# ERGO-Code/ipx

Hardware: AMD Instinct MI355X
Metric: kkt_solves_per_sec (higher is better)
Workload: dtype f64; 1 GPU; C3 synthetic LP m=1000000 n=2000000 8 nnz/col (nnz=16000000), KKTSolverDiag::Solve = diag-precond CR to tol=0.3*sqrt(mu), scaling spread s=1; rows of AI partitioned over 1 GPU(s); errflag=0

## Files before the change

include/ipx_kkt_hip.h:

```cpp
#ifndef IPX_KKT_HIP_H_
#define IPX_KKT_HIP_H_

#include <stdint.h>

#ifdef __cplusplus
extern "C" {
#endif

typedef int64_t ipxint;
typedef struct ipxk_context ipxk_context;

#define IPXK_OK 0
#define IPXK_E_HIP (-1)
#define IPXK_E_ALLOC (-2)
#define IPXK_E_ARGUMENT (-3)
#define IPXK_E_UNSUPPORTED (-4)

#define IPXK_POINTER_HOST 0
#define IPXK_POINTER_DEVICE 1

#define IPXK_NONBASIC_FIXED (-2)
#define IPXK_NONBASIC (-1)
#define IPXK_BASIC 0
#define IPXK_BASIC_FREE 1
// ... 50 lines not shown
int ipxk_get_reorder_info(const ipxk_context* ctx, ipxk_reorder_info* info);
int ipxk_get_reordering(ipxk_context* ctx, ipxint* rowperm, ipxint* colperm);
int ipxk_get_rowwise(const ipxk_context* ctx, ipxint* ATp, ipxint* ATi,
                     double* ATx);

int ipxk_normal_prepare(ipxk_context* ctx, const double* W);
int ipxk_normal_apply(ipxk_context* ctx, const double* rhs, double* lhs,
                      double* rhs_dot_lhs);

int ipxk_diag_factorize(ipxk_context* ctx, const double* W,
                        int precond_dense_cols, ipxint* errflag);
int ipxk_diag_apply(ipxk_context* ctx, const double* rhs, double* lhs,
                    double* rhs_dot_lhs);
int ipxk_diag_get(const ipxk_context* ctx, double* diagonal, double* chol);

typedef ipxint (*ipxk_interrupt_fn)(void* user);
int ipxk_pcr_solve(ipxk_context* ctx, const double* rhs, double tol,
                   const double* resscale, ipxint maxiter, double* lhs,
                   ipxint* iter, ipxint* errflag, ipxk_interrupt_fn interrupt,
                   void* interrupt_user, double* resnorm_hist, ipxint hist_cap,
                   ipxk_times* times);

int ipxk_cr_diagnostics(ipxk_context* ctx, ipxk_cr_diag* out);

int ipxk_kkt_diag_factorize(ipxk_context* ctx, const double* xl,
                            const double* xu, const double* zl,
                            const double* zu, double mu,
                            int precond_dense_cols, ipxint* errflag);
int ipxk_kkt_diag_solve(ipxk_context* ctx, const double* a, const double* b,
                        double tol, ipxint maxiter, double* x, double* y,
                        ipxint* iter, ipxint* errflag,
                        ipxk_interrupt_fn interrupt, void* interrupt_user,
                        ipxk_times* times);
int ipxk_kkt_diag_get(const ipxk_context* ctx, double* W, double* resscale);

int ipxk_split_prepare(ipxk_context* ctx, const ipxint* Lp, const ipxint* Li,
                       const double* Lx, const ipxint* Up, const ipxint* Ui,
                       const double* Ux, const ipxint* rowperm,
                       const ipxint* colperm, const ipxint* basis,
                       const ipxint* status, const double* colscale);
int ipxk_split_rescale(ipxk_context* ctx, const ipxint* status,
                       const double* colscale);
typedef struct {
  ipxint lnz, unz;
  ipxint num_dependent;
  ipxint col_singletons, row_singletons, bump, rounds;
// ... 262 lines not shown
```

ipx_amd/csrc/api.hip:

```cpp

#include <algorithm>
#include <map>
#include <thread>

#include "context.hpp"

namespace ipxk {

static thread_local std::string g_last_error;
void set_last_error(const std::string& msg) { g_last_error = msg; }

Context::~Context() {
    if (split) destroy_split(split);
    if (split_spare) destroy_split(split_spare);
    if (prepare_host) destroy_prepare_host(prepare_host);
    if (lu) destroy_lu(lu);
    if (maxvol) destroy_maxvol(maxvol);
    if (nmat) destroy_nmatrix(nmat);
    comm_destroy(this);
    if (h_state) (void)hipHostFree(h_state);
    if (h_cycle_done) (void)hipHostFree(h_cycle_done);
    if (ev_a) (void)hipEventDestroy(ev_a);
    if (ev_b) (void)hipEventDestroy(ev_b);
    for (hipEvent_t e : ev_window) (void)hipEventDestroy(e);
// ... 1008 lines not shown
        IPXK_REQUIRE(!comm_active(c), kDeviceLuRefusal);
        bind_device(c);
        maxvolume_dev(c, status, colscale, params, basis_out, status_out, info, exchange_log, log_cap);
    });
}

int ipxk_maxvolume_sequential(ipxk_context* c, const ipxint* status, const double* colscale, double volume_tol, ipxint maxpasses,
                              ipxint max_etas, ipxint* basis_out, ipxint* status_out, ipxk_maxvolume_info* info,
                              ipxint* exchange_log, ipxint log_cap) {
    return guarded([&] {
        IPXK_REQUIRE(c && status && colscale, "NULL argument");
        IPXK_REQUIRE(log_cap >= 0 && (exchange_log || log_cap == 0), "bad log arguments");
        IPXK_REQUIRE(!comm_active(c), kDeviceLuRefusal);
        bind_device(c);
        maxvolume_sequential_dev(c, status, colscale, volume_tol, maxpasses, max_etas, basis_out, status_out, info, exchange_log, log_cap);
    });
}

int ipxk_cr_diagnostics(ipxk_context* c, ipxk_cr_diag* out) {
    return guarded([&] {
        IPXK_REQUIRE(c && out, "NULL argument");
        bind_device(c);
        cr_diagnostics_dev(c, out);
    });
}

int ipxk_split_rescale(ipxk_context* c, const ipxint* status, const double* colscale) {
    return guarded([&] {
        IPXK_REQUIRE(c && status && colscale, "NULL argument");
        IPXK_REQUIRE(c->split != nullptr, "SplittedNormalMatrix not prepared");
        bind_device(c);
        split_rescale_host(c, status, colscale);
    });
}

int ipxk_split_apply(ipxk_context* c, const double* rhs, double* lhs, double* rhs_dot_lhs) {
    return guarded([&] {
        IPXK_REQUIRE(c && rhs && lhs, "NULL argument");
        IPXK_REQUIRE(c->split != nullptr, "SplittedNormalMatrix not prepared");
        split_check_partition(c);
        bind_device(c);
        if (c->partials.size() == 0) c->partials.resize((size_t)kNumPartialSlots * kPartialStride);
        const size_t m = (size_t)c->m;
        const double* drhs = stage_in(c, rhs, m, c->v_rhs);
        double* dlhs = stage_out(c, lhs, m, c->v_lhs);
        const int np = split_apply_dev(c, drhs, dlhs, nullptr);
// ... 264 lines not shown
```

ipx_amd/csrc/context.hpp:

```cpp
#pragma once

#include "internal.hpp"
#include "device_utils.hpp"

struct ncclComm;

namespace ipxk {

constexpr int kPartialStride = kMaxPartials + 8;

enum PartialSlot {
    kPartRes0 = 0,
    kPartRes1,
    kPartPdot,
    kPartCdot,
    kPartRsdot,
    kPartScratch,
    kNumPartialSlots
};

struct Reordered {
    bool active = false;
    int levels = 0;
    int components = 0;
// ... 49 lines not shown

    DevBuf<double> diagonal;
    bool diag_factorized = false;
    int64_t kdense = 0;
    GatherMatrix AdCols;
    GatherMatrix AdRows;
    DevBuf<double> chol, chol_inv, smw_work, smw_u, Wnodense;
    DevBuf<double> schur_panel, schur_part;
    DevBuf<int> schur_colptr;
    DevBuf<int> chol_info;
    DevBuf<unsigned char> dense_mask;
    std::vector<int> dense_rank_k;
    DevBuf<double> dense_W, dense_Wsend, dense_Wrecv;
    DevBuf<int> dense_Widx;

    DevBuf<double> v_rhs, v_lhs, v_residual, v_sresidual, v_step, v_Cstep, v_Cres, v_pCstep;
    DevBuf<double> v_resscale_in;
    DevBuf<double> partials;
    DevBuf<CrState> state;
    CrState* h_state = nullptr;
    DevBuf<double> hist;
    hipEvent_t ev_a = nullptr, ev_b = nullptr;
    std::vector<hipEvent_t> ev_window;

    DevBuf<double> resscale;
    DevBuf<double> k_a, k_b, k_x, k_y;
    DevBuf<double> k_tmp;
    bool kkt_diag_factorized = false;

    DevBuf<double> nw_rhs1, nw_rhs2;
    DevBuf<double> nw_in[10], nw_out[6];
    DevBuf<unsigned char> nw_state;

    DevBuf<double> it_x, it_xl, it_xu, it_y, it_zl, it_zu, it_partials;
    DevBuf<double> it_row, it_bnd, it_table;
    DevBuf<unsigned char> it_state;
    bool it_set = false;
    DevBuf<double> ipm[12];
    bool postprocessed = false;
    double crossover_start = 0.0;
    DevBuf<double> colmax;
    bool have_colmax = false;

    struct { long inverse_probes = 0, inverse_rejected = 0, inverse_refined = 0; double worst_probe = 0.0; } split_stats;
    SplitOperator* split = nullptr;
    SplitOperator* split_spare = nullptr;
// ... 57 lines not shown
void reorder_permute_rows(Context* c, const double* in_old, double* out_new);
void reorder_unpermute_rows(Context* c, const double* in_new, double* out_old);
void reorder_permute_weights(Context* c, const double* W_old, double* W_new);

void dense_lu_inverse(Context* c, int kb, const double* D, const double* invL, const double* invU, double* X, double* Xt, int refine = 0);

enum TimeKind { kTimeOp = 0, kTimePrecond = 1, kTimeB = 2, kTimeBt = 3, kNumTimeKinds = 4 };
void time_mark(Context* c, int kind, bool begin);
void time_start(Context* c, ipxk_times* times);
void time_collect(Context* c, ipxk_times* times);

const double* stage_in(Context* c, const double* p, size_t len, DevBuf<double>& buf);
double* stage_out(Context* c, double* p, size_t len, DevBuf<double>& buf);
void finish_out(Context* c, double* user, const double* dev, size_t len);

void normal_apply_dev(Context* c, const double* W, const double* rhs, double* lhs, int* ndot,
                      const int* done);
float time_normal_pair(Context* c, GatherMatrix& Ac, GatherMatrix& Ar);
void debug_single_pass(Context* c, int which, const double* x, double* out);

void prepare_dense_columns(Context* c);
void reset_dense_columns(Context* c);
void diag_factorize_dev(Context* c, const double* W, bool precond_dense_cols, ipxint* errflag);
int diag_apply_dev(Context* c, const double* rhs, double* lhs, int slot, const int* done);

struct CrResult { ipxint iter; ipxint errflag; };
CrResult pcr_solve_dev(Context* c, const double* rhs, double tol, const double* resscale,
                       ipxint maxiter, double* lhs, bool lhs_is_zero, ipxk_interrupt_fn interrupt,
                       void* user, double* hist_host, ipxint hist_cap, ipxk_times* times);
CrResult cr_solve_dev(Context* c, const double* rhs, double tol, const double* resscale,
                      ipxint maxiter, double* lhs, bool lhs_is_zero, ipxk_interrupt_fn interrupt,
                      void* user, double* hist_host, ipxint hist_cap, ipxk_times* times);
double reduce_partials_host(Context* c, int slot, int count, bool is_max);
void cr_diagnostics_dev(Context* c, ipxk_cr_diag* out);
struct PartRef publish_scalar(Context* c, int slot, int count, int op);
struct PartRef allreduce_scalar(Context* c, int slot, int count, int op);

CrResult newton_solve_dev(Context* c, bool use_basis, const double* rb, const double* rc, const double* rl,
                          const double* ru, const double* sl, const double* su, const double* xl, const double* xu,
                          const double* zl, const double* zu, const unsigned char* state, double tol,
                          ipxint maxiter, double* dx, double* dxl, double* dxu, double* dy, double* dzl,
                          double* dzu, ipxk_interrupt_fn interrupt, void* user, ipxk_times* times);

void iterate_update_dev(Context* c, double sp, const double* dx, const double* dxl, const double* dxu, double sd,
                        const double* dy, const double* dzl, const double* dzu);
void iterate_residuals_dev(Context* c, const double* b, const double* cc, const double* lb, const double* ub,
                           double* rb, double* rc, double* rl, double* ru, double* presidual, double* dresidual);
void iterate_complementarity_dev(Context* c, double out4[4], double* num_terms = nullptr);
enum IterWhat : unsigned { kIterResiduals = 1, kIterComplementarity = 2, kIterObjectives = 4 };
struct IterScalars {
    double presidual = 0, dresidual = 0;
    double comp[4] = {0, 0, 0, 0};
    double num_terms = 0;
    double obj[3] = {0, 0, 0};
};
void iterate_scalars_dev(Context* c, unsigned what, const double* b, const double* cc, const double* lb, const double* ub,
                         double* rb, double* rc, double* rl, double* ru, IterScalars* out);
// ... 155 lines not shown
```

ipx_amd/csrc/cr.hip:

```cpp
#include <cmath>

#include "context.hpp"
#include "spmv_kernels.hpp"

namespace ipxk {

constexpr int kWindow = 2;

enum CrMode { kModePcrDiag = 0, kModePcrSmw = 1, kModePlain = 2 };

constexpr int kCrUnroll = 4;

struct CrVecs {
    int m;
    double* lhs;
    double* residual;
    double* sresidual;
    double* step;
    double* Cstep;
    double* Cres;
    double* pCstep;
    const double* resscale;
    const double* diag;
};

__global__ __launch_bounds__(kBlock) void residual_init_kernel(int m, const double* __restrict__ rhs,
                                                               const double* __restrict__ sub,
                                                               const double* __restrict__ resscale,
                                                               double* __restrict__ out,
                                                               double* partial) {
// ... 160 lines not shown
    }

    double mx = 0.0;
    long long i0 = first;
    if (EARLY) {
        ctl_update<MODE>(v, lazy, alpha, i0, stride, last, g0, mx);
        i0 += kCrUnroll * stride;
    }
    for (; i0 < v.m; i0 += kCrUnroll * stride) {
        CtlGroup g{};
        ctl_load<MODE>(v, lazy, i0, stride, last, g);
        ctl_update<MODE>(v, lazy, alpha, i0, stride, last, g, mx);
    }
    mx = block_reduce<MaxOp>(mx, red);
    if (threadIdx.x == 0) ((k & 1) ? res_next0 : res_next1)[blockIdx.x] = mx;
    if (writer) {
        st->k_started = k + 1;
        st->resnorm = resnorm;
        if (lazy) { st->alpha_pending = alpha; st->k_pending = k; }
    }
}

struct DirGroup {
    double p[kCrUnroll], q[kCrUnroll], s[kCrUnroll], cs[kCrUnroll], d[kCrUnroll], l[kCrUnroll];
};
template <int MODE, bool INIT>
__device__ __forceinline__ void dir_load(const CrVecs& v, const double* src, bool with_lhs, long long i0, long long stride,
                                         long long last, DirGroup& g) {
#pragma unroll
    for (int u = 0; u < kCrUnroll; u++) {
        const long long i = min(i0 + u * stride, last);
        g.p[u] = src[i];
        g.q[u] = v.Cres[i];
        if (!INIT) { g.s[u] = v.step[i]; g.cs[u] = v.Cstep[i]; }
        if (MODE == kModePcrDiag) g.d[u] = v.diag[i];
        if (!INIT && with_lhs) g.l[u] = v.lhs[i];
    }
}
template <int MODE, bool INIT>
__device__ __forceinline__ void dir_update(const CrVecs& v, bool owed, double alpha, double beta, long long i0, long long stride,
                                           long long last, DirGroup& g, double& acc) {
#pragma unroll
    for (int u = 0; u < kCrUnroll; u++) {
        const long long i = i0 + u * stride;
        if (i > last) break;
        if (!INIT) {
            if (owed) v.lhs[i] = g.l[u] + alpha * g.s[u];
            g.p[u] = g.p[u] + beta * g.s[u];
            g.q[u] = g.q[u] + beta * g.cs[u];
        }
        v.step[i] = g.p[u];
        v.Cstep[i] = g.q[u];
        if (MODE == kModePcrDiag) acc += (g.q[u] / g.d[u]) * g.q[u];
        if (MODE == kModePlain) acc += g.q[u] * g.q[u];
    }
}

template <int MODE, bool INIT, bool EARLY>
__global__ __launch_bounds__(kBlock) void cr_direction_kernel(CrState* st, CrVecs v, PartRef cdot_ref,
                                                              double* pdot_partial) {
    __shared__ double red[kBlock / 64 + 1];
    const double* src = MODE == kModePlain ? v.residual : v.sresidual;
    const long long stride = (long long)gridDim.x * kBlock, last = v.m - 1;
    const long long first = blockIdx.x * kBlock + threadIdx.x;
    long long k;
    double cdotnew, beta, alpha;
    bool owed;
    DirGroup g0{};
    if (EARLY) {
        const int done = st->done;
        const long long k_started = st->k_started, k_pending = st->k_pending;
        const double cdot0 = st->cdot[0], cdot1 = st->cdot[1];
        alpha = st->alpha_pending;
        double pc[kPartialsPerThread];
        load_partials(cdot_ref, pc);
        dir_load<MODE, INIT>(v, src, true, first, stride, last, g0);
        cdotnew = block_reduce<SumOp>(fold_partials<SumOp>(cdot_ref, pc), red);
        if (done) return;
        k = INIT ? -1 : k_started - 1;
        beta = INIT ? 0.0 : cdotnew / ((k & 1) ? cdot1 : cdot0);
        owed = !INIT && k_pending == k;
    } else {
        if (st->done) return;
        k = INIT ? -1 : st->k_started - 1;
        cdotnew = reduce_partials<SumOp>(cdot_ref, red);
        beta = INIT ? 0.0 : cdotnew / st->cdot[k & 1];
        owed = !INIT && st->k_pending == k;
        alpha = st->alpha_pending;
    }
    double acc = 0.0;
    long long i0 = first;
    if (EARLY) {
        dir_update<MODE, INIT>(v, owed, alpha, beta, i0, stride, last, g0, acc);
        i0 += kCrUnroll * stride;
    }
    for (; i0 < v.m; i0 += kCrUnroll * stride) {
        DirGroup g{};
        dir_load<MODE, INIT>(v, src, owed, i0, stride, last, g);
        dir_update<MODE, INIT>(v, owed, alpha, beta, i0, stride, last, g, acc);
    }
    if (MODE != kModePcrSmw) {
        acc = block_reduce<SumOp>(acc, red);
        if (threadIdx.x == 0) pdot_partial[blockIdx.x] = acc;
    }
    if (blockIdx.x == 0 && threadIdx.x == 0) {
        st->cdot[(k + 1) & 1] = cdotnew;
        st->k_finished = k + 1;
    }
}

__global__ __launch_bounds__(kBlock) void cr_flush_update_kernel(const CrState* st, CrVecs v) {
    if (st->k_pending < 0 || st->k_pending != st->k_finished) return;
    const double alpha = st->alpha_pending;
    for (int i = blockIdx.x * kBlock + threadIdx.x; i < v.m; i += gridDim.x * kBlock) v.lhs[i] += alpha * v.step[i];
}

__global__ __launch_bounds__(kBlock) void finalize_scalar_kernel(PartRef ref, int op, double* out) {
    __shared__ double red[kBlock / 64 + 1];
    const double v = op == 1 ? reduce_partials<MaxOp>(ref, red)
                   : op == 2 ? reduce_partials<MinOp>(ref, red) : reduce_partials<SumOp>(ref, red);
    if (threadIdx.x == 0) *out = v;
}

__global__ void snapshot_done_kernel(const CrState* st, int* host_slot) {
    __hip_atomic_store(host_slot, st->done, __ATOMIC_RELAXED, __HIP_MEMORY_SCOPE_SYSTEM);
}
__global__ void cycle_flags_kernel(const CrState* st, double interrupt_flag, double* flags) {
    flags[0] = (double)st->done;
    flags[1] = interrupt_flag;
}
__global__ void snapshot_flags_kernel(const double* flags, int* host_done, int* host_interrupt) {
    __hip_atomic_store(host_interrupt, (int)flags[1], __ATOMIC_RELAXED, __HIP_MEMORY_SCOPE_SYSTEM);
    __hip_atomic_store(host_done, (int)flags[0], __ATOMIC_RELAXED, __HIP_MEMORY_SCOPE_SYSTEM);
}

constexpr int kDoneRing = kWindow + 2;
constexpr int kDoneNow = 2 * kDoneRing;

static bool cr_lazy() {
    static const bool setting = [] { const char* e = getenv("IPXK_CR_LAZY"); return !e || atoi(e) != 0; }();
    return setting;
}

static bool cr_early() {
    static const bool setting = [] { const char* e = getenv("IPXK_CR_EARLY"); return !e || atoi(e) != 0; }();
    return setting;
}

static int cr_grid_cap() {
    static const int setting = [] { const char* e = getenv("IPXK_CR_GRID"); return e ? atoi(e) : 0; }();
    return setting;
}

static void ensure_comm_buffers(Context* c) {
    if (c->comm_scalars.size() < 64) c->comm_scalars.resize(64);
    if (c->comm_send.size() < (size_t)kNumPartialSlots) {
        c->comm_send.resize(kNumPartialSlots);
        IPXK_HIP(hipMemsetAsync(c->comm_send.get(), 0, sizeof(double) * kNumPartialSlots, c->stream));
    }
    const size_t need = (size_t)c->nranks * kNumPartialSlots;
// ... 66 lines not shown
        IPXK_HIP(hipHostGetDevicePointer(reinterpret_cast<void**>(&c->d_cycle_done), c->h_cycle_done, 0));
    }
    while ((int)c->ev_window.size() < kWindow + 1) {
        hipEvent_t e;
        IPXK_HIP(hipEventCreateWithFlags(&e, hipEventDisableTiming));
        c->ev_window.push_back(e);
    }
}

struct CrOps {
    int mode;
    int (*applyC)(Context*, const double* rhs, double* lhs, const int* done);
};

static int applyC_normal(Context* c, const double* rhs, double* lhs, const int* done) {
    int np = 0;
    time_mark(c, kTimeOp, true);
    normal_apply_dev(c, c->W, rhs, lhs, &np, done);
    time_mark(c, kTimeOp, false);
    return np;
}
static int applyC_split(Context* c, const double* rhs, double* lhs, const int* done) {
    return split_apply_dev(c, rhs, lhs, done);
}

template <int MODE>
static CrResult run_cr(Context* c, const CrOps& ops, const double* rhs, double tol,
                       const double* resscale, ipxint maxiter, double* lhs, bool lhs_is_zero,
                       ipxk_interrupt_fn interrupt, void* user, double* hist_host, ipxint hist_cap,
                       ipxk_times* times) {
    ensure_workspaces(c);
    time_start(c, times);
    hipStream_t s = c->stream;
    const int m = (int)c->m;
    if (maxiter < 0) maxiter = (comm_active(c) ? c->m_global : c->m) + 100;
    if (hist_cap < 0) hist_cap = 0;
    if (!hist_host) hist_cap = 0;
    if (c->hist.size() < (size_t)hist_cap + 1) c->hist.resize((size_t)hist_cap + 1);
    CrState* st = c->state.get();
    int* done = &st->done;
    const int g = cr_grid_cap() > 0 ? std::min(vec_grid(m), cr_grid_cap()) : vec_grid(m);
    const Pub pub(c);
    for (int i = 0; i <= kDoneNow; i++) c->h_cycle_done[i] = 0;
    const bool multi = comm_active(c);
    const int lazy = cr_lazy() ? 1 : 0;
    const bool early = cr_early() && m > 0;
    const auto control = early ? cr_control_update_kernel<MODE, true> : cr_control_update_kernel<MODE, false>;
    const auto direction0 = early ? cr_direction_kernel<MODE, true, true> : cr_direction_kernel<MODE, true, false>;
    const auto direction = early ? cr_direction_kernel<MODE, false, true> : cr_direction_kernel<MODE, false, false>;
    int* done_now = multi ? nullptr : c->d_cycle_done + kDoneNow;
    if (multi) ensure_comm_buffers(c);

    CrVecs v;
    v.m = m; v.lhs = lhs; v.residual = c->v_residual.get(); v.sresidual = c->v_sresidual.get();
    v.step = c->v_step.get(); v.Cstep = c->v_Cstep.get(); v.Cres = c->v_Cres.get();
    v.pCstep = c->v_pCstep.get(); v.resscale = resscale; v.diag = c->reord.in_use ? c->reord.diagonal.get() : c->diagonal.get();

    IPXK_HIP(hipEventRecord(c->ev_a, s));

    if (lhs_is_zero) {
        hipLaunchKernelGGL(residual_init_kernel, dim3(g), dim3(kBlock), 0, s, m, rhs,
                           (const double*)nullptr, resscale, v.residual, c->part(kPartRes0));
    } else {
        ops.applyC(c, lhs, v.Cres, nullptr);
        hipLaunchKernelGGL(residual_init_kernel, dim3(g), dim3(kBlock), 0, s, m, rhs,
                           (const double*)v.Cres, resscale, v.residual, c->part(kPartRes0));
    }
    int nrsdot = 0;
    if (MODE != kModePlain) nrsdot = diag_apply_dev(c, v.residual, v.sresidual, kPartRsdot, nullptr);
    if (MODE != kModePlain) pub.publish(kPartRes0, g, 1, kPartRsdot, nrsdot, 0);
    else pub.publish(kPartRes0, g, 1);
    const PartRef res0 = pub.ref(kPartRes0, g), res1 = pub.ref(kPartRes1, g);
    const PartRef rsdot = MODE != kModePlain ? pub.ref(kPartRsdot, nrsdot) : PartRef{nullptr, 0, 1};
    hipLaunchKernelGGL(cr_init_state_kernel, dim3(1), dim3(kBlock), 0, s, st, tol, (long long)maxiter,
                       (long long)hist_cap, rsdot, (int)MODE);
    const double* csrc = MODE == kModePlain ? v.residual : v.sresidual;
    int ncdot = ops.applyC(c, csrc, v.Cres, nullptr);
    pub.publish(kPartCdot, ncdot, 0);
    hipLaunchKernelGGL(direction0, dim3(g), dim3(kBlock), 0, s, st, v,
                       pub.ref(kPartCdot, ncdot), c->part(kPartPdot));
    int npdot = g;
    if (MODE == kModePcrSmw) npdot = diag_apply_dev(c, v.Cstep, v.pCstep, kPartPdot, nullptr);
    pub.publish(kPartPdot, npdot, 0);
    const PartRef pdot_ref = pub.ref(kPartPdot, npdot);

    ipxint interrupt_flag = 0, my_interrupt = 0;
    bool agreed_done = false, tail = false;
    for (long long cycle = 0;; cycle++) {
        const long long k0 = cycle * 5;
        if (k0 > maxiter) break;
        if (cycle >= kWindow) {
            const long long cw = cycle - kWindow;
            IPXK_HIP(hipEventSynchronize(c->ev_window[cw % (kWindow + 1)]));
            if (*(volatile int*)(c->h_cycle_done + cw % kDoneRing)) { agreed_done = true; break; }
            if (multi) {
                const int agreed = *(volatile int*)(c->h_cycle_done + kDoneRing + cw % kDoneRing);
                if (agreed != 0) { interrupt_flag = agreed; break; }
            }
        }
        if (interrupt && cycle > 0) {
            my_interrupt = interrupt(user);
            if (!multi && my_interrupt != 0) { interrupt_flag = my_interrupt; break; }
        }
        for (long long k = k0; k < k0 + 5 && k <= maxiter; k++) {
            if (done_now && *(volatile int*)(c->h_cycle_done + kDoneNow)) tail = true;
            if (tail) break;
            hipLaunchKernelGGL(control, dim3(g), dim3(kBlock), 0, s, st, v,
                               res0, res1, pdot_ref, rsdot, c->part(kPartRes0), c->part(kPartRes1),
                               c->hist.get(), lazy, done_now);
            ncdot = ops.applyC(c, csrc, v.Cres, done);
            pub.publish(kPartCdot, ncdot, 0, ((k + 1) & 1) ? kPartRes1 : kPartRes0, g, 1);
            hipLaunchKernelGGL(direction, dim3(g), dim3(kBlock), 0, s, st, v,
                               pub.ref(kPartCdot, ncdot), c->part(kPartPdot));
            if (MODE == kModePcrSmw) diag_apply_dev(c, v.Cstep, v.pCstep, kPartPdot, done);
            if (MODE != kModePlain && (k + 1) % 5 == 0) {
                diag_apply_dev(c, v.residual, v.sresidual, kPartRsdot, done);
                pub.publish(kPartPdot, npdot, 0, kPartRsdot, nrsdot, 0);
            } else {
                pub.publish(kPartPdot, npdot, 0);
            }
        }
        if (multi) {
            double* flags = c->comm_scalars.get() + 56;
            hipLaunchKernelGGL(cycle_flags_kernel, dim3(1), dim3(1), 0, s, st, (double)my_interrupt, flags);
            comm_allreduce_max(c, flags, 2);
            hipLaunchKernelGGL(snapshot_flags_kernel, dim3(1), dim3(1), 0, s, flags, c->d_cycle_done + cycle % kDoneRing,
                               c->d_cycle_done + kDoneRing + cycle % kDoneRing);
        } else {
            hipLaunchKernelGGL(snapshot_done_kernel, dim3(1), dim3(1), 0, s, st, c->d_cycle_done + cycle % kDoneRing);
        }
        IPXK_HIP(hipEventRecord(c->ev_window[cycle % (kWindow + 1)], s));
    }
    if (lazy) hipLaunchKernelGGL(cr_flush_update_kernel, dim3(g), dim3(kBlock), 0, s, st, v);
    IPXK_HIP(hipEventRecord(c->ev_b, s));
    IPXK_HIP(hipMemcpyAsync(c->h_state, st, sizeof(CrState), hipMemcpyDeviceToHost, s));
    IPXK_HIP(hipStreamSynchronize(s));
    IPXK_HIP(hipGetLastError());
    comm_check(c);

    if (multi && agreed_done && !c->h_state->done)
        throw Error(IPXK_E_HIP, "ranks of a partitioned solve diverged (another rank finished the CR loop, this one did not)");
    CrResult res;
    if (c->h_state->done) {
        res.iter = c->h_state->iter;
        res.errflag = c->h_state->errflag;
    } else {
        res.iter = c->h_state->k_finished;
        res.errflag = interrupt_flag;
    }
    if (hist_cap > 0) {
        long long nh = c->h_state->done && c->h_state->errflag != 204 ? res.iter + 1 : res.iter;
        if (!c->h_state->done) nh = c->h_state->k_started;
        if (nh > hist_cap) nh = hist_cap;
        for (long long i = nh; i < hist_cap; i++) hist_host[i] = std::nan("");
        if (nh > 0) {
            c->hist.download(hist_host, (size_t)nh, s);
            IPXK_HIP(hipStreamSynchronize(s));
        }
    }
    if (times) {
        float ms = 0.f;
        IPXK_HIP(hipEventElapsedTime(&ms, c->ev_a, c->ev_b));
        times->cr = ms * 1e-3;
        time_collect(c, times);
// ... 12 lines not shown
void cr_diagnostics_dev(Context* c, ipxk_cr_diag* out) {
    *out = ipxk_cr_diag{};
    IPXK_REQUIRE(c->h_state != nullptr && c->state.size() > 0, "no CR run on this context yet");
    const CrState& st = *c->h_state;
    out->errflag = st.done ? st.errflag : 0;
    out->iter = st.done ? st.iter : st.k_finished;
    out->maxiter = st.maxiter;
    out->resnorm = st.resnorm;
    out->tol = st.tol;
    out->cdot = st.cdot[out->iter & 1];
    out->rps_old = st.diag_rps_old;
    out->rps_new = st.diag_rps_new;
    if (st.done && st.errflag == 202) {
        const int m = (int)c->m, g = vec_grid(m);
        auto norm = [&](const double* v) {
            hipLaunchKernelGGL(infnorm_partial_kernel, dim3(g), dim3(kBlock), 0, c->stream, m, v, c->part(kPartScratch));
            return reduce_partials_host(c, kPartScratch, g, true);
        };
        out->infnorm_residual = norm(c->v_residual.get());
        if (st.mode != kModePlain) out->infnorm_sresidual = norm(c->v_sresidual.get());
    }
}

CrResult pcr_solve_dev(Context* c, const double* rhs, double tol, const double* resscale,
                       ipxint maxiter, double* lhs, bool lhs_is_zero, ipxk_interrupt_fn interrupt,
                       void* user, double* hist_host, ipxint hist_cap, ipxk_times* times) {
    IPXK_REQUIRE(c->normal_prepared, "NormalMatrix not prepared");
    IPXK_REQUIRE(c->diag_factorized, "DiagonalPrecond not factorized");
    CrOps ops{c->kdense > 0 ? kModePcrSmw : kModePcrDiag, applyC_normal};
    if (c->kdense > 0)
        return run_cr<kModePcrSmw>(c, ops, rhs, tol, resscale, maxiter, lhs, lhs_is_zero, interrupt,
                                   user, hist_host, hist_cap, times);
    return run_cr<kModePcrDiag>(c, ops, rhs, tol, resscale, maxiter, lhs, lhs_is_zero, interrupt, user,
                                hist_host, hist_cap, times);
}

CrResult cr_solve_dev(Context* c, const double* rhs, double tol, const double* resscale,
                      ipxint maxiter, double* lhs, bool lhs_is_zero, ipxk_interrupt_fn interrupt,
                      void* user, double* hist_host, ipxint hist_cap, ipxk_times* times) {
    IPXK_REQUIRE(c->split != nullptr, "SplittedNormalMatrix not prepared");
    split_check_partition(c);
    CrOps ops{kModePlain, applyC_split};
    return run_cr<kModePlain>(c, ops, rhs, tol, resscale, maxiter, lhs, lhs_is_zero, interrupt, user,
                              hist_host, hist_cap, times);
}

// ... 2 lines not shown
```

ipx_amd/csrc/precond.hip:

```cpp
#include "context.hpp"
#include "spmv_kernels.hpp"

namespace ipxk {

__global__ __launch_bounds__(kBlock) void diag_apply_kernel(int m, const double* __restrict__ rhs,
                                                            const double* __restrict__ diag,
                                                            double* __restrict__ lhs,
                                                            double* partial, const int* done) {
    if (done && *done) return;
    __shared__ double red[kBlock / 64 + 1];
    double acc = 0.0;
    for (int i = blockIdx.x * kBlock + threadIdx.x; i < m; i += gridDim.x * kBlock) {
        const double r = rhs[i];
        const double l = r / diag[i];
        lhs[i] = l;
        acc += l * r;
    }
    acc = block_reduce<SumOp>(acc, red);
    if (threadIdx.x == 0) partial[blockIdx.x] = acc;
}

__global__ void divide_kernel(int m, const double* __restrict__ rhs, const double* __restrict__ diag,
                              double* __restrict__ u, const int* done) {
    if (done && *done) return;
// ... 502 lines not shown
                if (j1 < k) {
                    const int nt = (k - j1 + 63) / 64;
                    hipLaunchKernelGGL(cholesky_trailing_kernel, dim3(nt, nt), dim3(kBlock), 0, s, k, j0, j1, c->chol.get(),
                                       c->chol_info.get());
                }
            }
            c->chol_inv.ensure((size_t)((k + 63) / 64) * 64 * 64);
            hipLaunchKernelGGL(cholesky_invert_blocks_kernel, dim3((k + 63) / 64), dim3(64), 0, s, k, c->chol.get(), c->chol_inv.get());
        }
        int info = 0;
        c->chol_info.download(&info, 1, s);
        IPXK_HIP(hipStreamSynchronize(s));
        comm_check(c);
        if (info != 0) {
            *errflag = 401;
            return;
        }
        c->kdense = k;
    }
    IPXK_HIP(hipGetLastError());
    c->diag_factorized = true;
}

int diag_apply_dev(Context* c, const double* rhs, double* lhs, int slot, const int* done) {
    const int m = (int)c->m;
    hipStream_t s = c->stream;
    time_mark(c, kTimePrecond, true);
    struct EndMark { Context* c; ~EndMark() { time_mark(c, kTimePrecond, false); } } end_mark{c};
    if (c->kdense == 0) {
        const int g = vec_grid(m);
        hipLaunchKernelGGL(diag_apply_kernel, dim3(g), dim3(kBlock), 0, s, m, rhs,
                           c->reord.in_use ? c->reord.diagonal.get() : c->diagonal.get(), lhs, c->part(slot), done);
        return g;
    }
    const int k = (int)c->kdense;
    hipLaunchKernelGGL(divide_kernel, dim3(vec_grid(m)), dim3(kBlock), 0, s, m, rhs,
                       c->diagonal.get(), c->smw_u.get(), done);
    double* stage = comm_rows(c) ? comm_stage(c, (size_t)k) : nullptr;
    EpiScale es{{}, nullptr, stage ? stage : c->smw_work.get()};
    launch_spmv(c->AdCols, c->smw_u.get(), es, nullptr, done, s);
    if (stage) comm_allreduce_sum_staged(c, c->smw_work.get(), (size_t)k);
    else if (comm_rows(c)) comm_allreduce_sum(c, c->smw_work.get(), (size_t)k);
    if (k <= 64)
        hipLaunchKernelGGL(potrs_wave_kernel, dim3(1), dim3(64), 0, s, k, c->chol.get(),
                           c->smw_work.get(), done);
    else
        hipLaunchKernelGGL(potrs_blocked_kernel, dim3(1), dim3(1024), sizeof(double) * (k + 64), s, k,
                           c->chol.get(), c->chol_inv.get(), c->smw_work.get(), done);
    EpiSmwRows er{{}, rhs, c->diagonal.get(), lhs};
    return launch_spmv(c->AdRows, c->smw_work.get(), er, c->part(slot), done, s);
}

}
// ... 1 lines not shown
```

ipx_amd/kkt.py:

```python
import ctypes as C
import os
import subprocess

import numpy as np

HERE = os.path.dirname(os.path.abspath(__file__))
LIB_PATH = os.path.join(HERE, "lib", "libipx_kkt_hip.so")

i64, f64 = np.int64, np.float64
c_i64, c_f64 = C.c_int64, C.c_double
P_i64, P_f64 = C.POINTER(C.c_int64), C.POINTER(C.c_double)
INTERRUPT_FN = C.CFUNCTYPE(c_i64, C.c_void_p)

POINTER_HOST, POINTER_DEVICE = 0, 1
NONBASIC_FIXED, NONBASIC, BASIC, BASIC_FREE = -2, -1, 0, 1

EXPORTS = [
    "ipxk_last_error", "ipxk_device_count", "ipxk_create", "ipxk_destroy", "ipxk_set_pointer_mode",
    "ipxk_set_stream", "ipxk_synchronize", "ipxk_set_profiling", "ipxk_set_interrupt", "ipxk_reset_solver_state", "ipxk_get_reorder_info", "ipxk_get_reordering", "ipxk_num_dense_cols", "ipxk_get_rowwise",
    "ipxk_normal_prepare", "ipxk_normal_apply", "ipxk_diag_factorize", "ipxk_diag_apply",
    "ipxk_diag_get", "ipxk_pcr_solve", "ipxk_cr_diagnostics", "ipxk_kkt_diag_factorize", "ipxk_kkt_diag_solve",
    "ipxk_kkt_diag_get", "ipxk_split_prepare", "ipxk_split_rescale", "ipxk_split_apply", "ipxk_forward_solve",
    "ipxk_backward_solve", "ipxk_solve_dense", "ipxk_split_levels", "ipxk_cr_solve",
    "ipxk_kkt_basis_solve", "ipxk_newton_solve", "ipxk_iterate_set", "ipxk_iterate_get", "ipxk_iterate_update",
    "ipxk_iterate_residuals", "ipxk_iterate_complementarity", "ipxk_step_to_boundary", "ipxk_ipm_step", "ipxk_iterate_objectives", "ipxk_ipm_driver", "ipxk_iterate_factorize_diag", "ipxk_comm_unique_id", "ipxk_comm_init", "ipxk_comm_init_columns", "ipxk_comm_info", "ipxk_maxvolume_sequential",
    "ipxk_time_normal_apply", "ipxk_equilibrate", "ipxk_transpose", "ipxk_lu_factorize", "ipxk_lu_factorize_basis",
    "ipxk_lu_get_factors", "ipxk_lu_generation", "ipxk_split_prepare_lu", "ipxk_maxvolume", "ipxk_ipm_driver_basis",
    "ipxk_ipm_starting_point", "ipxk_ipm_load_starting_point", "ipxk_ipm_starting_basis", "ipxk_iterate_postprocess",
    "ipxk_iterate_dropping_residuals", "ipxk_ipm_set_crossover_start", "ipxk_iterate_drop_to_complementarity", "ipxk_ipm_solve",
    "ipxk_normal_apply_bytes", "ipxk_spmv_layout", "ipxk_layout_info", "ipxk_layout_array", "ipxk_split_inverse_stats", "ipxk_split_inverse_refined", "ipxk_dev_alloc", "ipxk_dev_free", "ipxk_dev_upload",
    "ipxk_dev_download",
    "ipxk_lp_create", "ipxk_lp_destroy", "ipxk_lp_context", "ipxk_lp_get_model", "ipxk_lp_solve", "ipxk_lp_postsolve", "ipxk_lp_evaluate",
    "ipxk_lp_get_residuals",
]


class IpmStepInfo(C.Structure):
    _fields_ = [("step_primal", c_f64), ("step_dual", c_f64), ("mu_before", c_f64), ("mu_after", c_f64),
                ("sigma", c_f64), ("presidual", c_f64), ("dresidual", c_f64), ("kktiter_predictor", c_i64),
                ("kktiter_corrector", c_i64), ("errflag", c_i64)]


class CrDiag(C.Structure):
    _fields_ = [("errflag", c_i64), ("iter", c_i64), ("maxiter", c_i64), ("resnorm", c_f64), ("tol", c_f64),
# ... 336 lines not shown
        return d, ch.reshape(k, k).T

    def _cr(self, fn, rhs, tol, resscale, maxiter, lhs0, hist_cap, interrupt):
        rhs = _F(rhs)
        lhs = np.zeros(self.m, f64) if lhs0 is None else _F(lhs0).copy()
        it, err = c_i64(0), c_i64(0)
        hist = np.full(max(hist_cap, 1), np.nan, f64)
        times = Times()
        cb = INTERRUPT_FN(lambda _u: int(interrupt())) if interrupt else C.cast(None, INTERRUPT_FN)
        self._check(fn(self.h, _fp(rhs), c_f64(tol), _fp(_F(resscale)), c_i64(maxiter), _fp(lhs),
                       C.byref(it), C.byref(err), cb, None, _fp(hist) if hist_cap else None,
                       c_i64(hist_cap), C.byref(times)))
        hist = hist[:hist_cap]
        return lhs, int(it.value), int(err.value), hist[~np.isnan(hist)], times

    def pcr_solve(self, rhs, tol, resscale, maxiter, lhs0=None, hist_cap=0, interrupt=None):
        return self._cr(self.lib.ipxk_pcr_solve, rhs, tol, resscale, maxiter, lhs0, hist_cap, interrupt)

    def cr_diagnostics(self):
        d = CrDiag()
        self._check(self.lib.ipxk_cr_diagnostics(self.h, C.byref(d)))
        return {k: getattr(d, k) for k, _ in CrDiag._fields_}

    def cr_solve(self, rhs, tol, resscale, maxiter, lhs0=None, hist_cap=0, interrupt=None):
        return self._cr(self.lib.ipxk_cr_solve, rhs, tol, resscale, maxiter, lhs0, hist_cap, interrupt)

    def kkt_diag_factorize(self, xl=None, xu=None, zl=None, zu=None, mu=0.0,
                           precond_dense_cols=True):
        err = c_i64(0)
        self._check(self.lib.ipxk_kkt_diag_factorize(
            self.h, _fp(_F(xl)), _fp(_F(xu)), _fp(_F(zl)), _fp(_F(zu)), c_f64(mu),
            C.c_int(1 if precond_dense_cols else 0), C.byref(err)))
        return int(err.value)

    def kkt_diag_solve(self, a, b, tol, maxiter=-1, interrupt=None):
        a, b = _F(a), _F(b)
        x, y = np.zeros(self.n + self.m, f64), np.zeros(self.m, f64)
        it, err, times = c_i64(0), c_i64(0), Times()
        cb = INTERRUPT_FN(lambda _u: int(interrupt())) if interrupt else C.cast(None, INTERRUPT_FN)
        self._check(self.lib.ipxk_kkt_diag_solve(self.h, _fp(a), _fp(b), c_f64(tol), c_i64(maxiter),
                                                 _fp(x), _fp(y), C.byref(it), C.byref(err), cb, None,
                                                 C.byref(times)))
        return x, y, int(it.value), int(err.value), times

    def kkt_diag_solve_resident(self, a_dev, b_dev, x_dev, y_dev, tol, maxiter=-1):
        it, err, times = c_i64(0), c_i64(0), Times()
# ... 383 lines not shown
```

Baseline: 64.63 solves/s.

## Pace CR loop by device progress counter and fuse residual refresh into direction kernel

Replaces the 5-iteration cycle pacing with snapshot kernels and event syncs in the single-GPU path. The host now polls a host-mapped progress word that the direction kernel writes each iteration, and keeps a fixed number of iterations enqueued ahead. This removes the per-cycle snapshot launch and event synchronisation, and lets the host stop enqueueing sooner after convergence. The periodic diagonal-preconditioner residual refresh is fused into the direction kernel, and diag_apply is launched on the CR grid. In exchange the host spins on a polled word, and a stalled-queue error path is added.

After: 65.63 solves/s, median of 6. 1.02x the previous value.

```diff
diff --git a/include/ipx_kkt_hip.h b/include/ipx_kkt_hip.h
--- a/include/ipx_kkt_hip.h
+++ b/include/ipx_kkt_hip.h
@@ -96,6 +96,7 @@
                    ipxk_times* times);
 
 int ipxk_cr_diagnostics(ipxk_context* ctx, ipxk_cr_diag* out);
+int ipxk_cr_loop_stats(ipxk_context* ctx, ipxint out[4]);
 
 int ipxk_kkt_diag_factorize(ipxk_context* ctx, const double* xl,
                             const double* xu, const double* zl,
diff --git a/ipx_amd/csrc/api.hip b/ipx_amd/csrc/api.hip
--- a/ipx_amd/csrc/api.hip
+++ b/ipx_amd/csrc/api.hip
@@ -1054,6 +1054,13 @@
         IPXK_REQUIRE(c && out, "NULL argument");
         bind_device(c);
         cr_diagnostics_dev(c, out);
+    });
+}
+
+int ipxk_cr_loop_stats(ipxk_context* c, ipxint out[4]) {
+    return guarded([&] {
+        IPXK_REQUIRE(c && out, "NULL argument");
+        cr_loop_stats_dev(c, out);
     });
 }
 
diff --git a/ipx_amd/csrc/context.hpp b/ipx_amd/csrc/context.hpp
--- a/ipx_amd/csrc/context.hpp
+++ b/ipx_amd/csrc/context.hpp
@@ -95,6 +95,7 @@
     DevBuf<double> hist;
     hipEvent_t ev_a = nullptr, ev_b = nullptr;
     std::vector<hipEvent_t> ev_window;
+    long long cr_loop_stats[4] = {0, 0, 0, 0};
 
     DevBuf<double> resscale;
     DevBuf<double> k_a, k_b, k_x, k_y;
@@ -198,7 +199,7 @@
 void prepare_dense_columns(Context* c);
 void reset_dense_columns(Context* c);
 void diag_factorize_dev(Context* c, const double* W, bool precond_dense_cols, ipxint* errflag);
-int diag_apply_dev(Context* c, const double* rhs, double* lhs, int slot, const int* done);
+int diag_apply_dev(Context* c, const double* rhs, double* lhs, int slot, const int* done, int grid = 0);
 
 struct CrResult { ipxint iter; ipxint errflag; };
 CrResult pcr_solve_dev(Context* c, const double* rhs, double tol, const double* resscale,
@@ -209,6 +210,7 @@
                       void* user, double* hist_host, ipxint hist_cap, ipxk_times* times);
 double reduce_partials_host(Context* c, int slot, int count, bool is_max);
 void cr_diagnostics_dev(Context* c, ipxk_cr_diag* out);
+void cr_loop_stats_dev(const Context* c, ipxint out[4]);
 struct PartRef publish_scalar(Context* c, int slot, int count, int op);
 struct PartRef allreduce_scalar(Context* c, int slot, int count, int op);
 
diff --git a/ipx_amd/csrc/cr.hip b/ipx_amd/csrc/cr.hip
--- a/ipx_amd/csrc/cr.hip
+++ b/ipx_amd/csrc/cr.hip
@@ -1,4 +1,8 @@
+#include <algorithm>
+#include <chrono>
 #include <cmath>
+#include <string>
+#include <thread>
 
 #include "context.hpp"
 #include "spmv_kernels.hpp"
@@ -6,6 +10,7 @@
 namespace ipxk {
 
 constexpr int kWindow = 2;
+constexpr int kAhead = 3;
 
 enum CrMode { kModePcrDiag = 0, kModePcrSmw = 1, kModePlain = 2 };
 
@@ -212,9 +217,9 @@
 }
 
 struct DirGroup {
-    double p[kCrUnroll], q[kCrUnroll], s[kCrUnroll], cs[kCrUnroll], d[kCrUnroll], l[kCrUnroll];
+    double p[kCrUnroll], q[kCrUnroll], s[kCrUnroll], cs[kCrUnroll], d[kCrUnroll], l[kCrUnroll], r[kCrUnroll];
 };
-template <int MODE, bool INIT>
+template <int MODE, bool INIT, bool REFRESH>
 __device__ __forceinline__ void dir_load(const CrVecs& v, const double* src, bool with_lhs, long long i0, long long stride,
                                          long long last, DirGroup& g) {
 #pragma unroll
@@ -225,11 +230,12 @@
         if (!INIT) { g.s[u] = v.step[i]; g.cs[u] = v.Cstep[i]; }
         if (MODE == kModePcrDiag) g.d[u] = v.diag[i];
         if (!INIT && with_lhs) g.l[u] = v.lhs[i];
-    }
-}
-template <int MODE, bool INIT>
+        if (REFRESH) g.r[u] = v.residual[i];
+    }
+}
+template <int MODE, bool INIT, bool REFRESH>
 __device__ __forceinline__ void dir_update(const CrVecs& v, bool owed, double alpha, double beta, long long i0, long long stride,
-                                           long long last, DirGroup& g, double& acc) {
+                                           long long last, DirGroup& g, double& acc, double& rs) {
 #pragma unroll
     for (int u = 0; u < kCrUnroll; u++) {
         const long long i = i0 + u * stride;
@@ -243,12 +249,19 @@
         v.Cstep[i] = g.q[u];
         if (MODE == kModePcrDiag) acc += (g.q[u] / g.d[u]) * g.q[u];
         if (MODE == kModePlain) acc += g.q[u] * g.q[u];
-    }
-}
-
-template <int MODE, bool INIT, bool EARLY>
+        if (REFRESH) {
+            const double l = g.r[u] / g.d[u];
+            v.sresidual[i] = l;
+            rs += l * g.r[u];
+        }
+    }
+}
+
+template <int MODE, bool INIT, bool EARLY, bool REFRESH>
 __global__ __launch_bounds__(kBlock) void cr_direction_kernel(CrState* st, CrVecs v, PartRef cdot_ref,
-                                                              double* pdot_partial) {
+                                                              double* pdot_partial, double* rsdot_partial,
+                                                              long long* host_progress) {
+    static_assert(!REFRESH || (MODE == kModePcrDiag && !INIT), "the fused refresh is the diagonal preconditioner's");
     __shared__ double red[kBlock / 64 + 1];
     const double* src = MODE == kModePlain ? v.residual : v.sresidual;
     const long long stride = (long long)gridDim.x * kBlock, last = v.m - 1;
@@ -264,7 +277,7 @@
         alpha = st->alpha_pending;
         double pc[kPartialsPerThread];
         load_partials(cdot_ref, pc);
-        dir_load<MODE, INIT>(v, src, true, first, stride, last, g0);
+        dir_load<MODE, INIT, REFRESH>(v, src, true, first, stride, last, g0);
         cdotnew = block_reduce<SumOp>(fold_partials<SumOp>(cdot_ref, pc), red);
         if (done) return;
         k = INIT ? -1 : k_started - 1;
@@ -279,23 +292,29 @@
         alpha = st->alpha_pending;
     }
     double acc = 0.0;
+    double rs = 0.0;
     long long i0 = first;
     if (EARLY) {
-        dir_update<MODE, INIT>(v, owed, alpha, beta, i0, stride, last, g0, acc);
+        dir_update<MODE, INIT, REFRESH>(v, owed, alpha, beta, i0, stride, last, g0, acc, rs);
         i0 += kCrUnroll * stride;
     }
     for (; i0 < v.m; i0 += kCrUnroll * stride) {
         DirGroup g{};
-        dir_load<MODE, INIT>(v, src, owed, i0, stride, last, g);
-        dir_update<MODE, INIT>(v, owed, alpha, beta, i0, stride, last, g, acc);
+        dir_load<MODE, INIT, REFRESH>(v, src, owed, i0, stride, last, g);
+        dir_update<MODE, INIT, REFRESH>(v, owed, alpha, beta, i0, stride, last, g, acc, rs);
     }
     if (MODE != kModePcrSmw) {
         acc = block_reduce<SumOp>(acc, red);
         if (threadIdx.x == 0) pdot_partial[blockIdx.x] = acc;
     }
+    if (REFRESH) {
+        rs = block_reduce<SumOp>(rs, red);
+        if (threadIdx.x == 0) rsdot_partial[blockIdx.x] = rs;
+    }
     if (blockIdx.x == 0 && threadIdx.x == 0) {
         st->cdot[(k + 1) & 1] = cdotnew;
         st->k_finished = k + 1;
+        if (host_progress) __hip_atomic_store(host_progress, k + 1, __ATOMIC_RELAXED, __HIP_MEMORY_SCOPE_SYSTEM);
     }
 }
 
@@ -326,6 +345,23 @@
 
 constexpr int kDoneRing = kWindow + 2;
 constexpr int kDoneNow = 2 * kDoneRing;
+constexpr int kProgress = kDoneNow + 2;
+static_assert(kProgress % 2 == 0 && kProgress + 2 <= 64, "the progress word lies inside h_cycle_done, aligned");
+
+static bool cr_pace_cycles() {
+    static const bool setting = [] { const char* e = getenv("IPXK_CR_PACE"); return e && std::string(e) == "cycles"; }();
+    return setting;
+}
+
+static long long cr_ahead() {
+    static const long long setting = [] { const char* e = getenv("IPXK_CR_AHEAD"); return e && atoi(e) > 0 ? atoi(e) : kAhead; }();
+    return setting;
+}
+
+static bool cr_refresh() {
+    static const bool setting = [] { const char* e = getenv("IPXK_CR_REFRESH"); return !e || atoi(e) != 0; }();
+    return setting;
+}
 
 static bool cr_lazy() {
     static const bool setting = [] { const char* e = getenv("IPXK_CR_LAZY"); return !e || atoi(e) != 0; }();
@@ -438,6 +474,29 @@
 }
 static int applyC_split(Context* c, const double* rhs, double* lhs, const int* done) {
     return split_apply_dev(c, rhs, lhs, done);
+}
+
+static bool wait_for_progress(Context* c, hipStream_t s, long long need) {
+    using clock = std::chrono::steady_clock;
+    constexpr std::chrono::microseconds kQueryAfter(2000), kQueryMax(128000);
+    const volatile int* done_now = c->h_cycle_done + kDoneNow;
+    const volatile long long* progress = reinterpret_cast<const volatile long long*>(c->h_cycle_done + kProgress);
+    if (*done_now || *progress >= need) return true;
+    clock::time_point asked = clock::now();
+    std::chrono::microseconds interval = kQueryAfter;
+    for (unsigned looks = 1;; looks++) {
+        std::this_thread::yield();
+        if (*done_now || *progress >= need) return true;
+        if (looks % 64 == 0 && clock::now() - asked >= interval) {
+            const hipError_t e = hipStreamQuery(s);
+            if (e != hipErrorNotReady) {
+                IPXK_HIP(e);
+                return *done_now || *progress >= need;
+            }
+            asked = clock::now();
+            interval = std::min(interval * 2, kQueryMax);
+        }
+    }
 }
 
 template <int MODE>
@@ -457,15 +516,24 @@
     int* done = &st->done;
     const int g = cr_grid_cap() > 0 ? std::min(vec_grid(m), cr_grid_cap()) : vec_grid(m);
     const Pub pub(c);
-    for (int i = 0; i <= kDoneNow; i++) c->h_cycle_done[i] = 0;
+    for (int i = 0; i < kProgress + 2; i++) c->h_cycle_done[i] = 0;
     const bool multi = comm_active(c);
     const int lazy = cr_lazy() ? 1 : 0;
     const bool early = cr_early() && m > 0;
     const auto control = early ? cr_control_update_kernel<MODE, true> : cr_control_update_kernel<MODE, false>;
-    const auto direction0 = early ? cr_direction_kernel<MODE, true, true> : cr_direction_kernel<MODE, true, false>;
-    const auto direction = early ? cr_direction_kernel<MODE, false, true> : cr_direction_kernel<MODE, false, false>;
+    const auto direction0 = early ? cr_direction_kernel<MODE, true, true, false> : cr_direction_kernel<MODE, true, false, false>;
+    const auto direction = early ? cr_direction_kernel<MODE, false, true, false> : cr_direction_kernel<MODE, false, false, false>;
+    auto direction5 = direction;
+    bool fused_refresh = false;
+    if constexpr (MODE == kModePcrDiag) {
+        fused_refresh = !multi && cr_refresh();
+        direction5 = early ? cr_direction_kernel<MODE, false, true, true> : cr_direction_kernel<MODE, false, false, true>;
+    }
     int* done_now = multi ? nullptr : c->d_cycle_done + kDoneNow;
+    long long* progress = multi ? nullptr : reinterpret_cast<long long*>(c->d_cycle_done + kProgress);
     if (multi) ensure_comm_buffers(c);
+    long long* stats = c->cr_loop_stats;
+    stats[0] = stats[1] = stats[2] = stats[3] = 0;
 
     CrVecs v;
     v.m = m; v.lhs = lhs; v.residual = c->v_residual.get(); v.sresidual = c->v_sresidual.get();
@@ -482,8 +550,10 @@
         hipLaunchKernelGGL(residual_init_kernel, dim3(g), dim3(kBlock), 0, s, m, rhs,
                            (const double*)v.Cres, resscale, v.residual, c->part(kPartRes0));
     }
+    stats[1]++;
     int nrsdot = 0;
-    if (MODE != kModePlain) nrsdot = diag_apply_dev(c, v.residual, v.sresidual, kPartRsdot, nullptr);
+    if (MODE != kModePlain) nrsdot = diag_apply_dev(c, v.residual, v.sresidual, kPartRsdot, nullptr, g);
+    if (MODE == kModePcrDiag) stats[1]++;
     if (MODE != kModePlain) pub.publish(kPartRes0, g, 1, kPartRsdot, nrsdot, 0);
     else pub.publish(kPartRes0, g, 1);
     const PartRef res0 = pub.ref(kPartRes0, g), res1 = pub.ref(kPartRes1, g);
@@ -494,60 +564,88 @@
     int ncdot = ops.applyC(c, csrc, v.Cres, nullptr);
     pub.publish(kPartCdot, ncdot, 0);
     hipLaunchKernelGGL(direction0, dim3(g), dim3(kBlock), 0, s, st, v,
-                       pub.ref(kPartCdot, ncdot), c->part(kPartPdot));
+                       pub.ref(kPartCdot, ncdot), c->part(kPartPdot), (double*)nullptr, progress);
+    stats[1] += 2;
     int npdot = g;
-    if (MODE == kModePcrSmw) npdot = diag_apply_dev(c, v.Cstep, v.pCstep, kPartPdot, nullptr);
+    if (MODE == kModePcrSmw) npdot = diag_apply_dev(c, v.Cstep, v.pCstep, kPartPdot, nullptr, g);
     pub.publish(kPartPdot, npdot, 0);
     const PartRef pdot_ref = pub.ref(kPartPdot, npdot);
 
+    const auto enqueue_iteration = [&](long long k) {
+        const bool refresh = MODE != kModePlain && (k + 1) % 5 == 0;
+        hipLaunchKernelGGL(control, dim3(g), dim3(kBlock), 0, s, st, v,
+                           res0, res1, pdot_ref, rsdot, c->part(kPartRes0), c->part(kPartRes1),
+                           c->hist.get(), lazy, done_now);
+        ncdot = ops.applyC(c, csrc, v.Cres, done);
+        pub.publish(kPartCdot, ncdot, 0, ((k + 1) & 1) ? kPartRes1 : kPartRes0, g, 1);
+        hipLaunchKernelGGL(refresh && fused_refresh ? direction5 : direction, dim3(g), dim3(kBlock), 0, s, st, v,
+                           pub.ref(kPartCdot, ncdot), c->part(kPartPdot), c->part(kPartRsdot), progress);
+        stats[0]++;
+        stats[1] += 2;
+        if (MODE == kModePcrSmw) diag_apply_dev(c, v.Cstep, v.pCstep, kPartPdot, done, g);
+        if (refresh && !fused_refresh) {
+            diag_apply_dev(c, v.residual, v.sresidual, kPartRsdot, done, g);
+            if (MODE == kModePcrDiag) stats[1]++;
+        }
+        if (refresh) pub.publish(kPartPdot, npdot, 0, kPartRsdot, nrsdot, 0);
+        else pub.publish(kPartPdot, npdot, 0);
+    };
+
     ipxint interrupt_flag = 0, my_interrupt = 0;
-    bool agreed_done = false, tail = false;
-    for (long long cycle = 0;; cycle++) {
-        const long long k0 = cycle * 5;
-        if (k0 > maxiter) break;
-        if (cycle >= kWindow) {
-            const long long cw = cycle - kWindow;
-            IPXK_HIP(hipEventSynchronize(c->ev_window[cw % (kWindow + 1)]));
-            if (*(volatile int*)(c->h_cycle_done + cw % kDoneRing)) { agreed_done = true; break; }
+    bool agreed_done = false, tail = false, stalled = false;
+    if (!multi && !cr_pace_cycles()) {
+        const long long R = cr_ahead();
+        for (long long k = 0; k <= maxiter; k++) {
+            if (!wait_for_progress(c, s, k - R)) { stalled = true; break; }
+            if (*(volatile int*)(c->h_cycle_done + kDoneNow)) break;
+            if (interrupt && k > 0 && k % 5 == 0) {
+                my_interrupt = interrupt(user);
+                if (my_interrupt != 0) { interrupt_flag = my_interrupt; break; }
+            }
+            enqueue_iteration(k);
+        }
+    } else {
+        for (long long cycle = 0;; cycle++) {
+            const long long k0 = cycle * 5;
+            if (k0 > maxiter) break;
+            if (cycle >= kWindow) {
+                const long long cw = cycle - kWindow;
+                IPXK_HIP(hipEventSynchronize(c->ev_window[cw % (kWindow + 1)]));
+                if (*(volatile int*)(c->h_cycle_done + cw % kDoneRing)) { agreed_done = true; break; }
+                if (multi) {
+                    const int agreed = *(volatile int*)(c->h_cycle_done + kDoneRing + cw % kDoneRing);
+                    if (agreed != 0) { interrupt_flag = agreed; break; }
+                }
+            }
+            if (interrupt && cycle > 0) {
+                my_interrupt = interrupt(user);
+                if (!multi && my_interrupt != 0) { interrupt_flag = my_interrupt; break; }
+            }
+            for (long long k = k0; k < k0 + 5 && k <= maxiter; k++) {
+                if (done_now && *(volatile int*)(c->h_cycle_done + kDoneNow)) tail = true;
+                if (tail) break;
+                enqueue_iteration(k);
+            }
             if (multi) {
-                const int agreed = *(volatile int*)(c->h_cycle_done + kDoneRing + cw % kDoneRing);
-                if (agreed != 0) { interrupt_flag = agreed; break; }
+                double* flags = c->comm_scalars.get() + 56;
+                hipLaunchKernelGGL(cycle_flags_kernel, dim3(1), dim3(1), 0, s, st, (double)my_interrupt, flags);
+                comm_allreduce_max(c, flags, 2);
+                hipLaunchKernelGGL(snapshot_flags_kernel, dim3(1), dim3(1), 0, s, flags, c->d_cycle_done + cycle % kDoneRing,
+                                   c->d_cycle_done + kDoneRing + cycle % kDoneRing);
+                stats[1] += 2;
+            } else {
+                hipLaunchKernelGGL(snapshot_done_kernel, dim3(1), dim3(1), 0, s, st, c->d_cycle_done + cycle % kDoneRing);
+                stats[1]++;
             }
-        }
-        if (interrupt && cycle > 0) {
-            my_interrupt = interrupt(user);
-            if (!multi && my_interrupt != 0) { interrupt_flag = my_interrupt; break; }
-        }
-        for (long long k = k0; k < k0 + 5 && k <= maxiter; k++) {
-            if (done_now && *(volatile int*)(c->h_cycle_done + kDoneNow)) tail = true;
-            if (tail) break;
-            hipLaunchKernelGGL(control, dim3(g), dim3(kBlock), 0, s, st, v,
-                               res0, res1, pdot_ref, rsdot, c->part(kPartRes0), c->part(kPartRes1),
-                               c->hist.get(), lazy, done_now);
-            ncdot = ops.applyC(c, csrc, v.Cres, done);
-            pub.publish(kPartCdot, ncdot, 0, ((k + 1) & 1) ? kPartRes1 : kPartRes0, g, 1);
-            hipLaunchKernelGGL(direction, dim3(g), dim3(kBlock), 0, s, st, v,
-                               pub.ref(kPartCdot, ncdot), c->part(kPartPdot));
-            if (MODE == kModePcrSmw) diag_apply_dev(c, v.Cstep, v.pCstep, kPartPdot, done);
-            if (MODE != kModePlain && (k + 1) % 5 == 0) {
-                diag_apply_dev(c, v.residual, v.sresidual, kPartRsdot, done);
-                pub.publish(kPartPdot, npdot, 0, kPartRsdot, nrsdot, 0);
-            } else {
-                pub.publish(kPartPdot, npdot, 0);
-            }
-        }
-        if (multi) {
-            double* flags = c->comm_scalars.get() + 56;
-            hipLaunchKernelGGL(cycle_flags_kernel, dim3(1), dim3(1), 0, s, st, (double)my_interrupt, flags);
-            comm_allreduce_max(c, flags, 2);
-            hipLaunchKernelGGL(snapshot_flags_kernel, dim3(1), dim3(1), 0, s, flags, c->d_cycle_done + cycle % kDoneRing,
-                               c->d_cycle_done + kDoneRing + cycle % kDoneRing);
-        } else {
-            hipLaunchKernelGGL(snapshot_done_kernel, dim3(1), dim3(1), 0, s, st, c->d_cycle_done + cycle % kDoneRing);
-        }
-        IPXK_HIP(hipEventRecord(c->ev_window[cycle % (kWindow + 1)], s));
-    }
-    if (lazy) hipLaunchKernelGGL(cr_flush_update_kernel, dim3(g), dim3(kBlock), 0, s, st, v);
+            stats[2]++;
+            IPXK_HIP(hipEventRecord(c->ev_window[cycle % (kWindow + 1)], s));
+            stats[3]++;
+        }
+    }
+    if (lazy) {
+        hipLaunchKernelGGL(cr_flush_update_kernel, dim3(g), dim3(kBlock), 0, s, st, v);
+        stats[1]++;
+    }
     IPXK_HIP(hipEventRecord(c->ev_b, s));
     IPXK_HIP(hipMemcpyAsync(c->h_state, st, sizeof(CrState), hipMemcpyDeviceToHost, s));
     IPXK_HIP(hipStreamSynchronize(s));
@@ -556,6 +654,8 @@
 
     if (multi && agreed_done && !c->h_state->done)
         throw Error(IPXK_E_HIP, "ranks of a partitioned solve diverged (another rank finished the CR loop, this one did not)");
+    if (stalled && !c->h_state->done)
+        throw Error(IPXK_E_HIP, "the CR loop's queue ran empty with iterations outstanding and the run not finished");
     CrResult res;
     if (c->h_state->done) {
         res.iter = c->h_state->iter;
@@ -614,6 +714,10 @@
     }
 }
 
+void cr_loop_stats_dev(const Context* c, ipxint out[4]) {
+    for (int i = 0; i < 4; i++) out[i] = (ipxint)c->cr_loop_stats[i];
+}
+
 CrResult pcr_solve_dev(Context* c, const double* rhs, double tol, const double* resscale,
                        ipxint maxiter, double* lhs, bool lhs_is_zero, ipxk_interrupt_fn interrupt,
                        void* user, double* hist_host, ipxint hist_cap, ipxk_times* times) {
diff --git a/ipx_amd/csrc/precond.hip b/ipx_amd/csrc/precond.hip
--- a/ipx_amd/csrc/precond.hip
+++ b/ipx_amd/csrc/precond.hip
@@ -548,13 +548,13 @@
     c->diag_factorized = true;
 }
 
-int diag_apply_dev(Context* c, const double* rhs, double* lhs, int slot, const int* done) {
+int diag_apply_dev(Context* c, const double* rhs, double* lhs, int slot, const int* done, int grid) {
     const int m = (int)c->m;
     hipStream_t s = c->stream;
     time_mark(c, kTimePrecond, true);
     struct EndMark { Context* c; ~EndMark() { time_mark(c, kTimePrecond, false); } } end_mark{c};
     if (c->kdense == 0) {
-        const int g = vec_grid(m);
+        const int g = grid > 0 ? grid : vec_grid(m);
         hipLaunchKernelGGL(diag_apply_kernel, dim3(g), dim3(kBlock), 0, s, m, rhs,
                            c->reord.in_use ? c->reord.diagonal.get() : c->diagonal.get(), lhs, c->part(slot), done);
         return g;
diff --git a/ipx_amd/kkt.py b/ipx_amd/kkt.py
--- a/ipx_amd/kkt.py
+++ b/ipx_amd/kkt.py
@@ -19,7 +19,7 @@
     "ipxk_last_error", "ipxk_device_count", "ipxk_create", "ipxk_destroy", "ipxk_set_pointer_mode",
     "ipxk_set_stream", "ipxk_synchronize", "ipxk_set_profiling", "ipxk_set_interrupt", "ipxk_reset_solver_state", "ipxk_get_reorder_info", "ipxk_get_reordering", "ipxk_num_dense_cols", "ipxk_get_rowwise",
     "ipxk_normal_prepare", "ipxk_normal_apply", "ipxk_diag_factorize", "ipxk_diag_apply",
-    "ipxk_diag_get", "ipxk_pcr_solve", "ipxk_cr_diagnostics", "ipxk_kkt_diag_factorize", "ipxk_kkt_diag_solve",
+    "ipxk_diag_get", "ipxk_pcr_solve", "ipxk_cr_diagnostics", "ipxk_cr_loop_stats", "ipxk_kkt_diag_factorize", "ipxk_kkt_diag_solve",
     "ipxk_kkt_diag_get", "ipxk_split_prepare", "ipxk_split_rescale", "ipxk_split_apply", "ipxk_forward_solve",
     "ipxk_backward_solve", "ipxk_solve_dense", "ipxk_split_levels", "ipxk_cr_solve",
     "ipxk_kkt_basis_solve", "ipxk_newton_solve", "ipxk_iterate_set", "ipxk_iterate_get", "ipxk_iterate_update",
@@ -402,6 +402,11 @@
         self._check(self.lib.ipxk_cr_diagnostics(self.h, C.byref(d)))
         return {k: getattr(d, k) for k, _ in CrDiag._fields_}
 
+    def cr_loop_stats(self):
+        out = np.zeros(4, i64)
+        self._check(self.lib.ipxk_cr_loop_stats(self.h, _ip(out)))
+        return {"iterations": int(out[0]), "launches": int(out[1]), "snapshots": int(out[2]), "events": int(out[3])}
+
     def cr_solve(self, rhs, tol, resscale, maxiter, lhs0=None, hist_cap=0, interrupt=None):
         return self._cr(self.lib.ipxk_cr_solve, rhs, tol, resscale, maxiter, lhs0, hist_cap, interrupt)
 
```
